# VITA-Group/SinNeRF

Hardware: AMD Instinct MI355X
Metric: rendered rays/sec (64+64 samples), lego 400x400 (higher is better)
Workload: dtype f32; 1 GPU; nerf_synthetic/lego-shaped 400x400 frame (160000 rays/GPU), N_samples=64, N_importance=64, eval render (perturb=0, noise_std=0, white_back), random-init teacher weights; points_per_ray=192, parallelism=rays sharded x1, no collective

## Files before the change

sinnerf_amd/csrc/sn_launch.h:

```cpp
#pragma once
#include <hip/hip_runtime.h>
#include <cstdlib>
#include "../../include/sinnerf_hip.h"
#include "sn_device.h"

namespace snh {

constexpr int MAX_DEVICES = 64;

inline int current_device() {
  int dev = 0;
  if (hipGetDevice(&dev) != hipSuccess || dev < 0 || dev >= MAX_DEVICES) return -1;
  return dev;
}

inline int cu_count() {
  static int cached[MAX_DEVICES];
  const int dev = current_device();
  if (dev < 0) return 256;
  int v = __atomic_load_n(&cached[dev], __ATOMIC_RELAXED);
  if (v == 0) {
    v = 256;
    (void)hipDeviceGetAttribute(&v, hipDeviceAttributeMultiprocessorCount, dev);
    __atomic_store_n(&cached[dev], v, __ATOMIC_RELAXED);
  }
  return v;
}

inline unsigned persistent_grid(long tiles) {
  const int n_cu = cu_count();
  return (unsigned)(tiles < n_cu ? tiles : n_cu);
}

#ifndef SN_DW_NARROW_ASM
#define SN_DW_NARROW_ASM 1
#endif
inline bool narrow_compiler_scheduled() {
  static const bool v = [] { const char* e = getenv("SINNERF_DW_NARROW_COMPILER"); return e != nullptr && e[0] == '1'; }();
  return v;
}
inline bool emb16_refused(int base_dtype, int emb16) {
  return emb16 && (base_dtype != SN_DTYPE_BF16_STATE || !SN_DW_NARROW_ASM || narrow_compiler_scheduled());
}

}

#define SN_ENSURE_DYN_LDS(KFN_, LDS_)                                                                               \
  do {                                                                                                              \
    static int sn_lds_set_[snh::MAX_DEVICES];                                                                       \
    const int sn_dev_ = snh::current_device();                                                                      \
    if (sn_dev_ < 0 || __atomic_load_n(&sn_lds_set_[sn_dev_], __ATOMIC_RELAXED) < (int)(LDS_)) {                    \
      hipError_t sn_e_ = hipFuncSetAttribute(reinterpret_cast<const void*>(KFN_),                                   \
                                             hipFuncAttributeMaxDynamicSharedMemorySize, (int)(LDS_));              \
      if (sn_e_ != hipSuccess) return (int)sn_e_;                                                                   \
      if (sn_dev_ >= 0) __atomic_store_n(&sn_lds_set_[sn_dev_], (int)(LDS_), __ATOMIC_RELAXED);                     \
    }                                                                                                               \
  } while (0)

namespace snd { struct Plan; }
extern "C" {
#define SN_FWD_PARAMS_                                                                                                              \
  const void* blob, const float* in0, const float* in1, long n_points, int s_or_ld, int sigma_only, int input_mode, float* out,    \
      float* acts, float* emb, long slot_rows
#define SN_CHAIN_PARAMS_                                                                                                            \
  const void* bblob, const float* acts, const float* out_raw, const float* g_raw, long n_points, long slot_rows, float* G, float* g_out
#define SN_RAYS_PARAMS_ const void* blob, const float* rays, const float* z_vals, long n_points, int n_samples, float* out
SN_DECLARE_HEADS(sn_mlp_forward_f32, (SN_FWD_PARAMS_, hipStream_t stream));
SN_DECLARE_HEADS(sn_mlp_forward_f32g, (SN_FWD_PARAMS_, hipStream_t stream));
SN_DECLARE_HEADS(sn_mlp_forward_f32g_store, (SN_FWD_PARAMS_, hipStream_t stream));
SN_DECLARE_HEADS(sn_mlp_forward_bf16x3, (SN_FWD_PARAMS_, hipStream_t stream));
SN_DECLARE_HEADS_F16(sn_mlp_forward_bf16, (SN_FWD_PARAMS_, int state_bf16, hipStream_t stream));
SN_DECLARE_HEADS_F16(sn_mlp_forward_bf16_v3, (SN_RAYS_PARAMS_, hipStream_t stream));
SN_DECLARE_HEADS(sn_mlp_forward_bf16_t, (SN_RAYS_PARAMS_, float* acts, float* emb, long slot_rows, int emb16, hipStream_t stream));
SN_DECLARE_HEADS(sn_mlp_forward_bf16x3_t, (SN_RAYS_PARAMS_, float* acts, float* emb, long slot_rows, hipStream_t stream));
SN_DECLARE_HEADS(sn_mlp_backward_chain_f32, (SN_CHAIN_PARAMS_, hipStream_t stream));
SN_DECLARE_HEADS(sn_mlp_backward_chain_f32g, (SN_CHAIN_PARAMS_, hipStream_t stream));
SN_DECLARE_HEADS(sn_mlp_backward_chain_bf16, (SN_CHAIN_PARAMS_, int state_bf16, hipStream_t stream));
SN_DECLARE_HEADS(sn_mlp_backward_chain_bf16_t, (SN_CHAIN_PARAMS_, hipStream_t stream));
SN_DECLARE_HEADS(sn_mlp_backward_chain_bf16x3, (SN_CHAIN_PARAMS_, hipStream_t stream));
SN_DECLARE_HEADS(sn_mlp_backward_chain_bf16x3_t, (SN_CHAIN_PARAMS_, hipStream_t stream));
#undef SN_FWD_PARAMS_
#undef SN_CHAIN_PARAMS_
#undef SN_RAYS_PARAMS_
int sn_dw_launch(const void* tasks, int n_tasks, hipStream_t stream);
long sn_weight_grads_workspace_bytes_impl(long slot_rows, int dtype, int emb16);
int sn_weight_grads_plan_impl(long slot_rows, int dtype, int emb16, int* out, int max_probs);
int sn_weight_grads_launch(const void* acts, const float* emb, const void* G, long slot_rows, int dtype, int emb16, void* workspace,
                           float* const* grads, int accumulate, hipStream_t stream);
int sn_dw_f32_asm_launch(const snd::Plan* plan_host, hipStream_t stream);
int sn_dw_bf16_asm_launch(const snd::Plan* plan_host, hipStream_t stream);
int sn_dw_narrow_bf16_asm_launch(const snd::Plan* plan_host, hipStream_t stream);
int sn_sample_coarse_launch(const float* rays, long n_rays, int n_samples, int use_disp, float perturb,
                            const float* perturb_rand, float* z_out, hipStream_t stream);
int sn_composite_forward_launch(const float* raw, int has_rgb, const float* z_vals, const float* rays,
                                const float* noise, float noise_std, long n_rays, int n_samples, int white_back,
                                float* rgb, float* depth, float* weights, hipStream_t stream);
int sn_composite_backward_launch(const float* raw, const float* z_vals, const float* rays, const float* noise,
                                 float noise_std, long n_rays, int n_samples, int white_back, const float* g_rgb,
                                 const float* g_depth, const float* g_w, float* g_raw, hipStream_t stream);
int sn_composite_backward_rays_launch(const float* raw, const float* z_vals, const float* rays, const float* noise,
                                      float noise_std, long n_rays, int n_samples, int white_back, const float* g_rgb,
                                      const float* g_depth, const float* g_w, float* g_raw, float* g_rays, hipStream_t stream);
int sn_sample_pdf_launch(const float* z_vals, const float* weights, const float* u, long n_rays, int n_samples,
                         int n_importance, float* z_fine, float* z_merged, hipStream_t stream);
int sn_sample_pdf_bins_launch(const float* bins, const float* weights, const float* u, long n_rays, int n_bins,
                              int n_importance, float eps, float* samples, hipStream_t stream);
int sn_generate_rays_launch(const float* c2w, int H, int W, float focal, float near, float far, int x0, int y0, int sx,
                            int sy, int pw, int ph, float* rays, hipStream_t stream);
long sn_generate_rays_backward_workspace_bytes_impl();
int sn_generate_rays_backward_launch(const float* g_rays, int H, int W, float focal, int x0, int y0, int sx, int sy, int pw,
                                     int ph, void* workspace, float* g_c2w, hipStream_t stream);
int sn_generate_rays_cam_launch(const float* c2w, float fx, float fy, float cx, float cy, int convention, int ndc, float ax, float ay,
                                float ndc_near, float near, float far, int x0, int y0, int sx, int sy, int pw, int ph, float* rays,
                                hipStream_t stream);
int sn_generate_rays_cam_backward_launch(const float* g_rays, const float* c2w, float fx, float fy, float cx, float cy, int convention,
                                         int ndc, float ax, float ay, float ndc_near, int x0, int y0, int sx, int sy, int pw, int ph,
                                         void* workspace, float* g_c2w, hipStream_t stream);
int sn_ndc_rays_launch(const float* rays_in, long n_rays, float ax, float ay, float ndc_near, float* rays_out, hipStream_t stream);
int sn_ndc_rays_backward_launch(const float* rays_in, const float* g_rays_out, long n_rays, float ax, float ay, float ndc_near,
                                float* g_rays_in, hipStream_t stream);
int sn_adam_step_launch(float* p, const float* g, float* m, float* v, long n, float lr, float b1, float b2, float eps,
                        float wd, int step, hipStream_t stream);
long sn_render_loss_workspace_bytes_impl();
int sn_render_loss_launch(const float* rgb_c, const float* rgb_f, const float* depth_c, const float* depth_f,
                          const float* rgb_gt, const float* depth_gt, const unsigned char* mask, int mask_mode, long n,
                          float w_rgb, float w_depth, float* g_rgb_c, float* g_rgb_f, float* g_depth_c, float* g_depth_f,
                          void* workspace, float* out, hipStream_t stream);
long sn_ray_grads_workspace_bytes_impl(long n_rays, int n_samples);
int sn_ray_grads_launch(const float* w1, const float* w5, const float* wdir, int layout, const void* g_acts, long slot_rows,
                        const float* rays, const float* z_vals, long n_rays, int n_samples, void* workspace, float* g_rays,
                        hipStream_t stream);
long sn_patch_loss_blocks_impl(int B, int H, int W, int C, int use_ssim);
long sn_patch_loss_workspace_bytes_impl(int B, int H, int W, int C, int use_ssim);
int sn_patch_loss_launch(const float* coarse, const float* fine, const float* target, int B, int H, int W, int C, int use_ssim, int window,
                         float w_mse, float w_ssim, float* g_coarse, float* g_fine, void* workspace, float* out, hipStream_t stream);
long sn_depth_smoothness_workspace_bytes_impl();
int sn_depth_smoothness_launch(const float* idepth, const float* image, int B, int H, int W, int C, float* g_idepth, float* g_image,
                               void* workspace, float* out, hipStream_t stream);
}
```

sinnerf_amd/csrc/sn_mlp_common.h:

```cpp
#pragma once
#include "sn_device.h"
#include "sn_layout.h"
#include "sn_launch.h"

namespace snk {

typedef __attribute__((address_space(3))) void lds_void;
typedef __attribute__((address_space(1))) const void gbl_cvoid;

__device__ __forceinline__ int slab_k_rt(int s) {
  return s < 8 ? snl::K_L0 : s < 32 ? snl::K_HID : s < 40 ? snl::K_SKIP : s < 72 ? snl::K_HID : snl::K_DIR;
}

SN_DEV f32x16 load_bias(const float* lds_bias, int s, int h) {
  const f32x4* p = reinterpret_cast<const f32x4*>(lds_bias + s * 32 + h * 16);
  f32x16 acc;
#pragma unroll
  for (int q = 0; q < 4; ++q) {
    const f32x4 v = p[q];
    acc[4 * q + 0] = v[0]; acc[4 * q + 1] = v[1]; acc[4 * q + 2] = v[2]; acc[4 * q + 3] = v[3];
  }
  return acc;
}

SN_DEV void embed_xyz(float x, float y, float z, int h, float* xe) {
  const Rev2 px = to_revolutions(x), py = to_revolutions(y), pz = to_revolutions(z);
  const float hs = h ? 32.0f : 1.0f;
#pragma unroll
  for (int p = 0; p < 15; ++p) {
    const Rev2 pc = (p % 3 == 0) ? px : (p % 3 == 1) ? py : pz;
    const float scale = hs * (float)(1 << (p / 3));
    sincos_rev(pc, scale, xe[2 * p], xe[2 * p + 1]);
  }
  xe[30] = h ? z : x;
  xe[31] = h ? 0.0f : y;
}
SN_DEV void embed_dir(float x, float y, float z, int h, float* de) {
  const Rev2 px = to_revolutions(x), py = to_revolutions(y), pz = to_revolutions(z);
  const float hs = h ? 4.0f : 1.0f;
#pragma unroll
  for (int p = 0; p < 6; ++p) {
    const Rev2 pc = (p % 3 == 0) ? px : (p % 3 == 1) ? py : pz;
    const float scale = hs * (float)(1 << (p / 3));
    sincos_rev(pc, scale, de[2 * p], de[2 * p + 1]);
  }
  de[12] = h ? z : x;
  de[13] = h ? 0.0f : y;
  de[14] = 0.0f;
  de[15] = 0.0f;
}


constexpr int xyz_col_slot(int k) { return 2 * (3 * (k / 6) + k % 3) + (k % 6) / 3; }
SN_DEV void store_emb_xyz(float* er, const float* f, int h) {
  float* base = er + 3 + 30 * h;
#pragma unroll
  for (int q = 0; q < 7; ++q) {
    f32x4 v;
#pragma unroll
    for (int i = 0; i < 4; ++i) v[i] = f[xyz_col_slot(4 * q + i)];
    __builtin_memcpy(base + 4 * q, &v, 16);
  }
  base[28] = f[xyz_col_slot(28)];
  base[29] = f[xyz_col_slot(29)];
  er[h ? 2 : 0] = f[30];
  if (!h) er[1] = f[31];
}
constexpr int dir_col_slot(int k) { return 2 * (3 * (k / 6) + k % 3) + (k % 6) / 3; }
SN_DEV void store_emb_dir(float* er64, const float* f, int h) {
  float* base = er64 + 3 + 12 * h;
#pragma unroll
  for (int q = 0; q < 3; ++q) {
    f32x4 v;
#pragma unroll
    for (int i = 0; i < 4; ++i) v[i] = f[dir_col_slot(4 * q + i)];
    __builtin_memcpy(base + 4 * q, &v, 16);
  }
  er64[h ? 2 : 0] = f[12];
  if (!h) er64[1] = f[13];
}

SN_DEV void sincos_double(float s, float c, float& s2, float& c2) {
  const float ts = s + s;
  s2 = ts * c;
  c2 = __builtin_fmaf(-ts, s, 1.0f);
}
SN_DEV void embed_xyz_dbl(float x, float y, float z, int h, float* xe) {
  const Rev2 px = to_revolutions(x), py = to_revolutions(y), pz = to_revolutions(z);
  const float hs = h ? 32.0f : 1.0f;
  sincos_rev(px, hs, xe[0], xe[1]);
  sincos_rev(py, hs, xe[2], xe[3]);
  sincos_rev(pz, hs, xe[4], xe[5]);
#pragma unroll
  for (int p = 3; p < 15; ++p) sincos_double(xe[2 * (p - 3)], xe[2 * (p - 3) + 1], xe[2 * p], xe[2 * p + 1]);
  xe[30] = h ? z : x;
  xe[31] = h ? 0.0f : y;
}
SN_DEV void embed_dir_dbl(float x, float y, float z, int h, float* de) {
  const Rev2 px = to_revolutions(x), py = to_revolutions(y), pz = to_revolutions(z);
  const float hs = h ? 4.0f : 1.0f;
  sincos_rev(px, hs, de[0], de[1]);
  sincos_rev(py, hs, de[2], de[3]);
  sincos_rev(pz, hs, de[4], de[5]);
#pragma unroll
  for (int p = 3; p < 6; ++p) sincos_double(de[2 * (p - 3)], de[2 * (p - 3) + 1], de[2 * p], de[2 * p + 1]);
  de[12] = h ? z : x;
  de[13] = h ? 0.0f : y;
  de[14] = 0.0f;
  de[15] = 0.0f;
}
#ifndef SN_EMBED_DBL
#define SN_EMBED_DBL 1
#endif
SN_DEV void embed_xyz_bf16(float x, float y, float z, int h, float* xe) {
  if (SN_EMBED_DBL) embed_xyz_dbl(x, y, z, h, xe); else embed_xyz(x, y, z, h, xe);
}
SN_DEV void embed_dir_bf16(float x, float y, float z, int h, float* de) {
  if (SN_EMBED_DBL) embed_dir_dbl(x, y, z, h, de); else embed_dir(x, y, z, h, de);
}

}
```

sinnerf_amd/csrc/sn_mlp_f32g.h:

```cpp
#pragma once
#include "sn_mlp_pipe.h"
#include <type_traits>

namespace snk {

#ifndef SN_F32G_FD
#define SN_F32G_FD 8
#endif
constexpr int FD_INFER = SN_F32G_FD;
#ifndef SN_F32G_FD_STORE
#define SN_F32G_FD_STORE 16
#endif
constexpr int FD_STORE = SN_F32G_FD_STORE;
constexpr int EPI_STEPS = 24, EPI_STEPS_STORE = 30;
#ifndef SN_F32G_WAIT_G
#define SN_F32G_WAIT_G 6
#endif
constexpr int F32G_LDS_BYTES = TAIL_LDS_BYTES + EPI_LDS_BYTES;
constexpr int F32G_LDS_BYTES_STORE = TAIL_LDS_BYTES + XPOSE_LDS_BYTES;

typedef __amdgpu_buffer_rsrc_t rsrc_t;

SN_DEV f32x4 load_frag(rsrc_t rs, unsigned voff, unsigned soff) {
  typedef unsigned u32x4 __attribute__((ext_vector_type(4)));
  const u32x4 v = __builtin_amdgcn_raw_buffer_load_b128(rs, voff, soff, 0);
  return __builtin_bit_cast(f32x4, v);
}

template <int NG0, int NG1, int SET0, int SET1, int G0, int TOT, int NSTEPS, int FD, class Pending>
SN_DEV void slab_f32g(f32x16& acc, f32x16& accn, f32x4 (&fr)[FD], rsrc_t rs, unsigned voff,
                      const float* bv, const float* lds_bias, int s_next, int h, Pending&& pending) {
  constexpr int NG = NG0 + NG1;
  static_assert(NG % 4 == 0 && TOT % FD == 0 && NG >= 8, "ring index = stream index mod FD");
#pragma unroll
  for (int g = 0; g < NG; ++g) {
    if (g == 0 || g == 12) asm volatile("s_waitcnt lgkmcnt(0)" ::: "memory");
    if (g == 6) accn = load_bias(lds_bias, s_next, h);
    __builtin_amdgcn_sched_barrier(0);
    const f32x4 a_cur = fr[(G0 + g) % FD];
    auto mma = [&](int kk) __attribute__((always_inline)) {
      if (g == 0 && kk == 0) {
        if (SET0 < 0) mma32_v<true>(acc, a_cur[0], bv[0]); else mma32_a<true>(acc, a_cur[0], SET0 * 128);
      } else if (g < NG0) {
        if (SET0 < 0) mma32_v<false>(acc, a_cur[kk], bv[4 * g + kk]); else mma32_a<false>(acc, a_cur[kk], SET0 * 128 + 4 * g + kk);
      } else {
        if (SET1 < 0) mma32_v<false>(acc, a_cur[kk], bv[4 * (g - NG0) + kk]);
        else mma32_a<false>(acc, a_cur[kk], SET1 * 128 + 4 * (g - NG0) + kk);
      }
    };
    auto step = [&](int kk) __attribute__((always_inline)) {
      const int st = 4 * g + kk - 2;
      if (st >= 0 && st < NSTEPS) pending(st);
    };
    mma(0);
    __builtin_amdgcn_sched_barrier(0);
    step(0);
    __builtin_amdgcn_sched_barrier(0);
    mma(1);
    __builtin_amdgcn_sched_barrier(0);
    fr[(G0 + g - 1 + FD) % FD] = load_frag(rs, voff, (unsigned)((G0 + g - 1 + FD) % TOT) * 1024u);
    step(1);
    __builtin_amdgcn_sched_barrier(0);
    mma(2);
    __builtin_amdgcn_sched_barrier(0);
    step(2);
    __builtin_amdgcn_sched_barrier(0);
    mma(3);
    __builtin_amdgcn_sched_barrier(0);
    step(3);
  }
}


}
```

sinnerf_amd/csrc/sn_mlp_fwd_f32g.hip:

```cpp
#include "sn_mlp_f32g.h"

namespace snk {

constexpr unsigned slab_byte_offset(int s) { return (unsigned)(snl::slab_elem_offset(s) * 4); }

template <bool SIGMA_ONLY, int INPUT_MODE, bool STORE>
__global__ void __launch_bounds__(256)
mlp_fwd_f32g_kernel(const char* __restrict__ blob, const float* __restrict__ in0, const float* __restrict__ in1, long P, int S,
                    float* __restrict__ out, float* __restrict__ acts, float* __restrict__ emb, long slot_rows) {
  constexpr int FD = STORE ? FD_STORE : FD_INFER;
  constexpr int NSTEPS = STORE ? EPI_STEPS_STORE : EPI_STEPS;
  extern __shared__ __attribute__((aligned(16))) char smem[];
  float* lds_bias = reinterpret_cast<float*>(smem);
  const float* lds_aux = lds_bias + snl::BIAS_FLOATS;

  const int tid = threadIdx.x;
  const int lane = tid & 63;
  const int wave = tid >> 6;
  const int j = lane & 31;
  const int h = lane >> 5;
  const long n_tiles = (P + 127) / 128;
  constexpr int N_USED = SIGMA_ONLY ? snl::SLAB_FIN : snl::N_SLABS;

  {
    const float4* gb = reinterpret_cast<const float4*>(blob + snl::bias_byte_offset(snl::DT_F32));
    float4* lb = reinterpret_cast<float4*>(lds_bias);
    for (int i = tid; i < snl::TAIL_FLOATS / 4; i += 256) lb[i] = gb[i];
  }
  __syncthreads();

  asm volatile("" ::: "a0", "a255");
  const rsrc_t rs = __builtin_amdgcn_make_buffer_rsrc(const_cast<char*>(blob), 0, (int)snl::blob_bytes(snl::DT_F32), 0x00020000);
  unsigned voff = lane * 16;
  asm volatile("" : "+v"(voff));
  f32x4 fr[FD];
#pragma unroll
  for (int g = 0; g < FD - 1; ++g) fr[g] = load_frag(rs, voff, g * 1024);
  f32x16 acc0 = load_bias(lds_bias, 0, h), acc1;
  char* const xp = smem + TAIL_LDS_BYTES + wave * XPOSE_WAVE_BYTES;
  const unsigned xp_w = (unsigned)(j * XPOSE_PITCH + 4 * h) * 4u;
  const unsigned xp_r = (unsigned)((lane >> 3) * XPOSE_PITCH + 4 * (lane & 7)) * 4u;
  unsigned g_off = (unsigned)((lane >> 3) * 256 + 4 * (lane & 7)) * 4u;
  constexpr int EQ = STORE ? 32 : 1024;
  unsigned epi_a = STORE ? (unsigned)(size_t)xp + xp_w : (unsigned)(size_t)(smem + TAIL_LDS_BYTES + wave * EPI_WAVE_BYTES) + lane * 16;
  asm volatile("" : "+v"(g_off));
  f32x4 rowbuf[2];
  unsigned vzero;
  asm volatile("v_mov_b32 %0, 0" : "=v"(vzero));
  asm volatile("" : "+v"(epi_a));

  for (long tile = blockIdx.x; tile < n_tiles; tile += gridDim.x) {
  const long p_wave = (tile * 4 + __builtin_amdgcn_readfirstlane(wave)) * 32;
  const long p_raw = p_wave + j;
  const bool valid = p_raw < P;
  const long p = valid ? p_raw : P - 1;

  float xe[32];
  if (INPUT_MODE == 0) {
#ifdef SN_F32G_NO_RAY_LOADS
    const float ox = 0.1f, oy = 0.2f, oz = 0.3f, dx = 0.5f, dy = 0.4f, dz = -0.7f, zz = 2.0f + 1e-6f * (float)p;
#else
    const long ray = p / S;
    const float* rp = in0 + ray * 8;
    const float ox = rp[0], oy = rp[1], oz = rp[2], dx = rp[3], dy = rp[4], dz = rp[5];
    const float zz = in1[p];
#endif
    const float x = __fadd_rn(ox, __fmul_rn(dx, zz));
    const float y = __fadd_rn(oy, __fmul_rn(dy, zz));
    const float z = __fadd_rn(oz, __fmul_rn(dz, zz));
#ifdef SN_F32G_NO_VALU_BLOCKS
#pragma unroll
    for (int e = 0; e < 32; ++e) xe[e] = x + (float)e;
#else
    embed_xyz(x, y, z, h, xe);
#endif
  } else {
    const float* row = in0 + p * (long)S;
    int hh = h;
    asm volatile("" : "+v"(hh));
#pragma unroll
    for (int e = 0; e < 32; ++e) {
      const int c0 = snl::xyz_slot_col(0, e), c1 = snl::xyz_slot_col(1, e);
      const int c = hh ? c1 : c0;
      xe[e] = (c >= 0) ? row[c < 0 ? 0 : c] : 0.0f;
    }
  }

  if (STORE && INPUT_MODE == 0) {
    int hh = h;
    asm volatile("" : "+v"(hh));
    store_emb_xyz(emb + p_raw * 128, xe, hh);
  }

  float sg = 0.0f;
  float sv[16];

  auto quad = [](const f32x16& r, int q) __attribute__((always_inline)) {
    f32x4 x;
    x[0] = r[4 * q]; x[1] = r[4 * q + 1]; x[2] = r[4 * q + 2]; x[3] = r[4 * q + 3];
    return x;
  };
  const long p_wave_c = p_wave;
  auto row_read = [&](int i) __attribute__((always_inline)) {
    return *reinterpret_cast<const f32x4*>(xp + xp_r + 8 * i * XPOSE_PITCH * 4);
  };
  auto row_store = [&](int slot, int t, int i, const f32x4& o) __attribute__((always_inline)) {
    const char* base = reinterpret_cast<const char*>(acts) + (((long)slot * slot_rows + p_wave_c + 8 * i) * 256 + 32 * t) * 4;
#ifdef SN_F32G_NO_ROW_STORES
    asm volatile("" :: "v"(o), "s"(base), "v"(g_off));
#else
    __builtin_nontemporal_store(o, reinterpret_cast<f32x4*>(const_cast<char*>(base) + g_off));
#endif
  };
  auto row_step = [&](int slot, int t, int k) __attribute__((always_inline)) {
    if (!STORE) return;
    if (k == 0) rowbuf[0] = row_read(0);
    else if (k == 1) rowbuf[1] = row_read(1);
    else if (k == 2) { row_store(slot, t, 0, rowbuf[0]); rowbuf[0] = row_read(2); }
    else if (k == 3) { row_store(slot, t, 1, rowbuf[1]); rowbuf[1] = row_read(3); }
    else if (k == 4) row_store(slot, t, 2, rowbuf[0]);
    else if (k == 5) row_store(slot, t, 3, rowbuf[1]);
  };
  f32x4 sw[4];
  auto relu_prog = [&](auto wset, auto slot_c, int t, int st, const f32x16& r) __attribute__((always_inline)) {
    constexpr int W = decltype(wset)::value;
    constexpr int slot = decltype(slot_c)::value;
    const int q = st / 6, k = st % 6;
    if (slot == 7) {
      if (st == 0) {
#pragma unroll
        for (int i = 0; i < 4; ++i) sw[i] = *reinterpret_cast<const f32x4*>(lds_aux + snl::AUX_SIGW + h * 128 + 16 * t + 4 * i);
      } else if (st == 3) {
#ifdef SN_F32G_NO_VALU_BLOCKS
#pragma unroll
        for (int i = 0; i < 16; ++i) sv[i] = r[i];
        if (false)
#endif
#pragma unroll
        for (int i = 0; i < 16; ++i) sv[i] = relu1(r[i]);
#pragma unroll
#ifndef SN_F32G_NO_VALU_BLOCKS
        for (int i = 0; i < 16; ++i) sg = __builtin_fmaf(sw[i / 4][i % 4], sv[i], sg);
#else
        for (int i = 0; i < 1; ++i) sg += sv[0];
#endif
        asm volatile("" : "+v"(sg));
      } else if (st >= 4 && st < 8) {
        f32x4 x;
        x[0] = sv[4 * (st - 4)]; x[1] = sv[4 * (st - 4) + 1]; x[2] = sv[4 * (st - 4) + 2]; x[3] = sv[4 * (st - 4) + 3];
        lds_put_quad(epi_a, EQ * (st - 4), x);
      } else if (st >= 8 && st < 12) {
        lds_get_quad_agpr(W * 128 + 16 * t + 4 * (st - 8), epi_a, EQ * (st - 8));
      } else if (st >= 24) {
        row_step(7, t, st - 24);
      }
      return;
    }
    if (st >= 24) { row_step(slot, t, st - 24); return; }
    if (k == 0) lds_put_quad(epi_a, EQ * q, quad(r, q));
#ifndef SN_F32G_NO_ATOMICS
    else if (k < 5) lds_relu_word(epi_a, EQ * q + 4 * (k - 1), vzero);
#endif
    else if (k == 5) lds_get_quad_agpr(W * 128 + 16 * t + 4 * q, epi_a, EQ * q);
  };
  auto copy_prog = [&](auto wset, auto, int t, int st, const f32x16& r) __attribute__((always_inline)) {
    constexpr int W = decltype(wset)::value;
    const int q = st / 6, k = st % 6;
    if (st >= 24) { row_step(8, t, st - 24); return; }
    if (k == 0) lds_put_quad(epi_a, EQ * q, quad(r, q));
    else if (k == 5) lds_get_quad_agpr(W * 128 + 16 * t + 4 * q, epi_a, EQ * q);
  };
  auto no_prog = [&](auto, auto, int, int, const f32x16&) __attribute__((always_inline)) {};

#define SN_C(V_) std::integral_constant<int, V_>{}
#define SN_SLABG(S_, NG0_, NG1_, S0_, S1_, BV_, PEPI_, PW_, PSLOT_, PT_)                                                  \
  do {                                                                                                                    \
    constexpr int s_nx = ((S_) + 1 == N_USED) ? 0 : (S_) + 1;                                                             \
    constexpr int g0 = (int)(slab_byte_offset(S_) / 1024), tot = (int)(slab_byte_offset(N_USED) / 1024);                  \
    if (((S_) & 1) == 0)                                                                                                  \
      slab_f32g<NG0_, NG1_, S0_, S1_, g0, tot, NSTEPS, FD>(acc0, acc1, fr, rs, voff, BV_,                                             \
          lds_bias, s_nx, h, [&](int st) __attribute__((always_inline)) { PEPI_(SN_C(PW_), SN_C(PSLOT_), PT_, st, acc1); }); \
    else                                                                                                                  \
      slab_f32g<NG0_, NG1_, S0_, S1_, g0, tot, NSTEPS, FD>(acc1, acc0, fr, rs, voff, BV_,                                             \
          lds_bias, s_nx, h, [&](int st) __attribute__((always_inline)) { PEPI_(SN_C(PW_), SN_C(PSLOT_), PT_, st, acc0); }); \
  } while (0)
#define SN_LAYERG(L_, NG0_, NG1_, S0_, S1_, EPI_, W_, PEPI_, PW_, PSLOT_)                 \
  do {                                                                                    \
    SN_SLABG(8 * (L_) + 0, NG0_, NG1_, S0_, S1_, xe, PEPI_, PW_, PSLOT_, 7);              \
    SN_SLABG(8 * (L_) + 1, NG0_, NG1_, S0_, S1_, xe, EPI_, W_, L_, 0);                    \
    SN_SLABG(8 * (L_) + 2, NG0_, NG1_, S0_, S1_, xe, EPI_, W_, L_, 1);                    \
    SN_SLABG(8 * (L_) + 3, NG0_, NG1_, S0_, S1_, xe, EPI_, W_, L_, 2);                    \
    SN_SLABG(8 * (L_) + 4, NG0_, NG1_, S0_, S1_, xe, EPI_, W_, L_, 3);                    \
    SN_SLABG(8 * (L_) + 5, NG0_, NG1_, S0_, S1_, xe, EPI_, W_, L_, 4);                    \
    SN_SLABG(8 * (L_) + 6, NG0_, NG1_, S0_, S1_, xe, EPI_, W_, L_, 5);                    \
    SN_SLABG(8 * (L_) + 7, NG0_, NG1_, S0_, S1_, xe, EPI_, W_, L_, 6);                    \
  } while (0)

  SN_LAYERG(0, 8, 0, -1, -1, relu_prog, 0, no_prog, 0, 0);
  SN_LAYERG(1, 32, 0, 0, 0, relu_prog, 1, relu_prog, 0, 0);
  SN_LAYERG(2, 32, 0, 1, 1, relu_prog, 0, relu_prog, 1, 1);
  SN_LAYERG(3, 32, 0, 0, 0, relu_prog, 1, relu_prog, 0, 2);
  SN_LAYERG(4, 8, 32, -1, 1, relu_prog, 0, relu_prog, 1, 3);
  SN_LAYERG(5, 32, 0, 0, 0, relu_prog, 1, relu_prog, 0, 4);
  SN_LAYERG(6, 32, 0, 1, 1, relu_prog, 0, relu_prog, 1, 5);
  SN_LAYERG(7, 32, 0, 0, 0, relu_prog, 1, relu_prog, 0, 6);

  if (SIGMA_ONLY) {
    mfma32_result_fence(acc1);
#pragma unroll
    for (int st = 0; st < EPI_STEPS; ++st) relu_prog(SN_C(1), SN_C(7), 7, st, acc1);
    const float sigma = sg + __shfl_xor(sg, 32, 64) + lds_aux[snl::AUX_HEADB];
    if (valid && h == 0) out[p_raw] = sigma;
    continue;
  }

  SN_LAYERG(8, 32, 0, 1, 1, copy_prog, 0, relu_prog, 1, 7);
  const float sigma = sg + __shfl_xor(sg, 32, 64) + lds_aux[snl::AUX_HEADB];

  float de[16];
  if (INPUT_MODE == 0) {
    const float* rp = in0 + (p / S) * 8;
#ifdef SN_F32G_NO_VALU_BLOCKS
#pragma unroll
    for (int e = 0; e < 16; ++e) de[e] = rp[3] + (float)e;
#else
    embed_dir(rp[3], rp[4], rp[5], h, de);
#endif
  } else {
    const float* row = in0 + p * (long)S;
    int hh = h;
    asm volatile("" : "+v"(hh));
#pragma unroll
    for (int e = 0; e < 16; ++e) {
      const int c0 = snl::dir_slot_col(0, e), c1 = snl::dir_slot_col(1, e);
      const int c = hh ? c1 : c0;
      de[e] = (c >= 0) ? row[63 + (c < 0 ? 0 : c)] : 0.0f;
    }
  }
  if (STORE && INPUT_MODE == 0) {
    int hh = h;
    asm volatile("" : "+v"(hh));
    store_emb_dir(emb + p_raw * 128 + 64, de, hh);
  }
  float c3[3] = {0.0f, 0.0f, 0.0f};
  auto ssp_slice = [&](auto, auto, int t, int st, const f32x16& r) __attribute__((always_inline)) {
    if (st >= 24) { row_step(9, t, st - 24); return; }
    if (st % 6 != 0) return;
    const int q = st / 6;
    float v[4];
#pragma unroll
#ifdef SN_F32G_NO_VALU_BLOCKS
    for (int i = 0; i < 4; ++i) v[i] = r[4 * q + i];
#else
    for (int i = 0; i < 4; ++i) v[i] = SN_NEWACT ? shifted_softplus_fast(r[4 * q + i]) : relu1(r[4 * q + i]);
#endif
#pragma unroll
#ifdef SN_F32G_NO_VALU_BLOCKS
    for (int c = 0; c < 1; ++c) c3[0] += v[0];
    if (false)
#endif
    for (int c = 0; c < 3; ++c) {
      const f32x4 w = *reinterpret_cast<const f32x4*>(lds_aux + snl::AUX_RGBW + c * 128 + h * 64 + 16 * t + 4 * q);
      c3[c] = __builtin_fmaf(w[0], v[0], c3[c]);
      c3[c] = __builtin_fmaf(w[1], v[1], c3[c]);
      c3[c] = __builtin_fmaf(w[2], v[2], c3[c]);
      c3[c] = __builtin_fmaf(w[3], v[3], c3[c]);
    }
    asm volatile("" : "+v"(c3[0]), "+v"(c3[1]), "+v"(c3[2]));
    if (STORE) {
      f32x4 o;
      o[0] = v[0]; o[1] = v[1]; o[2] = v[2]; o[3] = v[3];
      *reinterpret_cast<f32x4*>(xp + xp_w + 32 * q) = o;
    }
  };
  SN_SLABG(72, 32, 4, 0, -1, de, copy_prog, 0, 8, 7);
  SN_SLABG(73, 32, 4, 0, -1, de, ssp_slice, 0, 9, 0);
  SN_SLABG(74, 32, 4, 0, -1, de, ssp_slice, 0, 9, 1);
  SN_SLABG(75, 32, 4, 0, -1, de, ssp_slice, 0, 9, 2);
  mfma32_result_fence(acc1);
#pragma unroll
  for (int q = 0; q < 4; ++q) ssp_slice(SN_C(0), SN_C(9), 3, 6 * q, acc1);
  if (STORE) {
#pragma unroll
    for (int i = 0; i < 4; ++i) row_store(9, 3, i, row_read(i));
  }

  {
    float o3[3];
#pragma unroll
    for (int c = 0; c < 3; ++c) o3[c] = c3[c] + __shfl_xor(c3[c], 32, 64) + lds_aux[snl::AUX_HEADB + 1 + c];
    if (valid && h == 0) {
      float4 o;
      o.x = rgb_activation(o3[0]);
      o.y = rgb_activation(o3[1]);
      o.z = rgb_activation(o3[2]);
      o.w = sigma;
      reinterpret_cast<float4*>(out)[p_raw] = o;
    }
  }
  }
#undef SN_C
#undef SN_SLABG
#undef SN_LAYERG
}

}

#ifdef SN_F32G_TU_STORE
#define SN_F32G_ENTRY sn_mlp_forward_f32g_store
#else
#define SN_F32G_ENTRY sn_mlp_forward_f32g
#endif
#define SN_F32G_LAUNCH_NAME(base) SN_LAUNCH_NAME(base)
extern "C" int SN_F32G_LAUNCH_NAME(SN_F32G_ENTRY)(const void* blob, const float* in0, const float* in1, long n_points, int s_or_ld,
                                             int sigma_only, int input_mode, float* out, float* acts, float* emb, long slot_rows,
                                             hipStream_t stream) {
  using namespace snk;
  if (n_points <= 0) return 0;
  const long tiles = (n_points + 127) / 128;
  const bool store = acts != nullptr;
  if (store && (sigma_only || emb == nullptr || slot_rows < tiles * 128)) return SN_E_BADARG;
  dim3 grid(snh::persistent_grid(tiles)), block(256);
  const size_t lds = store ? F32G_LDS_BYTES_STORE : F32G_LDS_BYTES;
  const char* b = reinterpret_cast<const char*>(blob);
#define SN_LAUNCH(SO, IM, ST)                                                                                       \
  do {                                                                                                              \
    auto kfn = mlp_fwd_f32g_kernel<SO, IM, ST>;                                                                     \
    SN_ENSURE_DYN_LDS(kfn, lds);                                                                                    \
    hipLaunchKernelGGL(kfn, grid, block, lds, stream, b, in0, in1, n_points, s_or_ld, out, acts, emb, slot_rows);   \
  } while (0)
#if defined(SN_F32G_AB)
#ifdef SN_F32G_AB_STORE
  if (!store || input_mode != 0) return SN_E_UNSUPPORTED;
  SN_LAUNCH(false, 0, true);
#else
  if (store || sigma_only || input_mode != 0) return SN_E_UNSUPPORTED;
  SN_LAUNCH(false, 0, false);
#endif
#elif defined(SN_F32G_TU_STORE)
  if (!store) return SN_E_UNSUPPORTED;
  if (input_mode == 0) SN_LAUNCH(false, 0, true); else SN_LAUNCH(false, 1, true);
#elif defined(SN_CLASSIC_HEADS)
  if (store || sigma_only) return SN_E_UNSUPPORTED;
  if (input_mode == 0) SN_LAUNCH(false, 0, false); else SN_LAUNCH(false, 1, false);
#else
  if (store) return SN_E_UNSUPPORTED;
  if (input_mode == 0) { if (sigma_only) SN_LAUNCH(true, 0, false); else SN_LAUNCH(false, 0, false); }
  else { if (sigma_only) SN_LAUNCH(true, 1, false); else SN_LAUNCH(false, 1, false); }
#endif
#undef SN_LAUNCH
  return (int)hipGetLastError();
}
```

Before: 660,900 rays/s.

## Switch f32g inference to per-wave dynamic work stealing with cheaper ray indexing

Replaces the static per-block tile loop with per-wave 32-point units handed out through a global atomic ticket counter that is reset per stream before each launch. The goal is to even out load imbalance across CUs at the tail. It also swaps the 64-bit per-lane p/S division for a per-wave magic-multiply division plus a carry. When a wave's 32 points all share one ray, the direction embedding is computed once across lanes and broadcast through LDS. The cost is an extra memset per launch, an atomic per unit, more LDS, a host-side mutex-guarded map lookup per call, and a hard limit on the number of streams.

Result: faster. 668,500 rays/s, median of 6 (+1.2%).

```diff
diff --git a/sinnerf_amd/csrc/sn_launch.h b/sinnerf_amd/csrc/sn_launch.h
--- a/sinnerf_amd/csrc/sn_launch.h
+++ b/sinnerf_amd/csrc/sn_launch.h
@@ -1,6 +1,8 @@
 #pragma once
 #include <hip/hip_runtime.h>
 #include <cstdlib>
+#include <mutex>
+#include <unordered_map>
 #include "../../include/sinnerf_hip.h"
 #include "sn_device.h"
 
@@ -30,6 +32,21 @@
 inline unsigned persistent_grid(long tiles) {
   const int n_cu = cu_count();
   return (unsigned)(tiles < n_cu ? tiles : n_cu);
+}
+
+constexpr int UNIT_WORDS = 1024;
+inline int unit_word(hipStream_t stream) {
+  static std::mutex mu;
+  static std::unordered_map<hipStream_t, int> of[MAX_DEVICES];
+  const int dev = current_device();
+  if (dev < 0) return -1;
+  std::lock_guard<std::mutex> lock(mu);
+  auto it = of[dev].find(stream);
+  if (it != of[dev].end()) return it->second;
+  const int w = (int)of[dev].size();
+  if (w >= UNIT_WORDS) return -1;
+  of[dev].emplace(stream, w);
+  return w;
 }
 
 #ifndef SN_DW_NARROW_ASM
diff --git a/sinnerf_amd/csrc/sn_mlp_common.h b/sinnerf_amd/csrc/sn_mlp_common.h
--- a/sinnerf_amd/csrc/sn_mlp_common.h
+++ b/sinnerf_amd/csrc/sn_mlp_common.h
@@ -48,6 +48,26 @@
   de[13] = h ? 0.0f : y;
   de[14] = 0.0f;
   de[15] = 0.0f;
+}
+constexpr int DIR_LINE_FLOATS = 32;
+SN_DEV void embed_dir_shared(float x, float y, float z, int lane, float* line, float* de) {
+  const int L = lane < 12 ? lane : 0;
+  const int hh = L >= 6 ? 1 : 0, p = L - 6 * hh, c = p >= 3 ? p - 3 : p;
+  const float v = c == 0 ? x : c == 1 ? y : z;
+  const float scale = (hh ? 4.0f : 1.0f) * (p >= 3 ? 2.0f : 1.0f);
+  float2 sc;
+  sincos_rev(to_revolutions(v), scale, sc.x, sc.y);
+  if (lane < 12) *reinterpret_cast<float2*>(line + 16 * hh + 2 * p) = sc;
+  else if (lane == 12) *reinterpret_cast<float4*>(line + 12) = make_float4(x, y, 0.0f, 0.0f);
+  else if (lane == 13) *reinterpret_cast<float4*>(line + 28) = make_float4(z, 0.0f, 0.0f, 0.0f);
+  __builtin_amdgcn_wave_barrier();
+  const float4* src = reinterpret_cast<const float4*>(line + 16 * (lane >> 5));
+#pragma unroll
+  for (int q = 0; q < 4; ++q) {
+    const float4 t = src[q];
+    de[4 * q] = t.x; de[4 * q + 1] = t.y; de[4 * q + 2] = t.z; de[4 * q + 3] = t.w;
+  }
+  __builtin_amdgcn_wave_barrier();
 }
 
 
diff --git a/sinnerf_amd/csrc/sn_mlp_f32g.h b/sinnerf_amd/csrc/sn_mlp_f32g.h
--- a/sinnerf_amd/csrc/sn_mlp_f32g.h
+++ b/sinnerf_amd/csrc/sn_mlp_f32g.h
@@ -16,7 +16,7 @@
 #ifndef SN_F32G_WAIT_G
 #define SN_F32G_WAIT_G 6
 #endif
-constexpr int F32G_LDS_BYTES = TAIL_LDS_BYTES + EPI_LDS_BYTES;
+constexpr int F32G_LDS_BYTES = TAIL_LDS_BYTES + EPI_LDS_BYTES + 4 * DIR_LINE_FLOATS * 4;
 constexpr int F32G_LDS_BYTES_STORE = TAIL_LDS_BYTES + XPOSE_LDS_BYTES;
 
 typedef __amdgpu_buffer_rsrc_t rsrc_t;
diff --git a/sinnerf_amd/csrc/sn_mlp_fwd_f32g.hip b/sinnerf_amd/csrc/sn_mlp_fwd_f32g.hip
--- a/sinnerf_amd/csrc/sn_mlp_fwd_f32g.hip
+++ b/sinnerf_amd/csrc/sn_mlp_fwd_f32g.hip
@@ -1,13 +1,25 @@
 #include "sn_mlp_f32g.h"
+#include "sn_ray_index.h"
+
+#ifdef SN_F32G_STAMP_EXIT
+#define SN_F32G_STAMP_PARAM , unsigned long* __restrict__ stamp
+#define SN_F32G_STAMP_ARG , sn_f32g_stamp_buffer
+#else
+#define SN_F32G_STAMP_PARAM
+#define SN_F32G_STAMP_ARG
+#endif
 
 namespace snk {
+
+__device__ unsigned f32g_unit_words[snh::UNIT_WORDS];
 
 constexpr unsigned slab_byte_offset(int s) { return (unsigned)(snl::slab_elem_offset(s) * 4); }
 
 template <bool SIGMA_ONLY, int INPUT_MODE, bool STORE>
 __global__ void __launch_bounds__(256)
 mlp_fwd_f32g_kernel(const char* __restrict__ blob, const float* __restrict__ in0, const float* __restrict__ in1, long P, int S,
-                    float* __restrict__ out, float* __restrict__ acts, float* __restrict__ emb, long slot_rows) {
+                    float* __restrict__ out, float* __restrict__ acts, float* __restrict__ emb, long slot_rows,
+                    unsigned unit_word, unsigned long ray_m, unsigned ray_sh SN_F32G_STAMP_PARAM) {
   constexpr int FD = STORE ? FD_STORE : FD_INFER;
   constexpr int NSTEPS = STORE ? EPI_STEPS_STORE : EPI_STEPS;
   extern __shared__ __attribute__((aligned(16))) char smem[];
@@ -19,7 +31,12 @@
   const int wave = tid >> 6;
   const int j = lane & 31;
   const int h = lane >> 5;
-  const long n_tiles = (P + 127) / 128;
+#ifdef SN_F32G_STATIC_UNITS
+  constexpr bool DYN = false;
+#else
+  constexpr bool DYN = !STORE;
+#endif
+  const long n_units = STORE ? (P + 127) / 128 * 4 : (P + 31) / 32;
   constexpr int N_USED = SIGMA_ONLY ? snl::SLAB_FIN : snl::N_SLABS;
 
   {
@@ -34,8 +51,6 @@
   unsigned voff = lane * 16;
   asm volatile("" : "+v"(voff));
   f32x4 fr[FD];
-#pragma unroll
-  for (int g = 0; g < FD - 1; ++g) fr[g] = load_frag(rs, voff, g * 1024);
   f32x16 acc0 = load_bias(lds_bias, 0, h), acc1;
   char* const xp = smem + TAIL_LDS_BYTES + wave * XPOSE_WAVE_BYTES;
   const unsigned xp_w = (unsigned)(j * XPOSE_PITCH + 4 * h) * 4u;
@@ -48,22 +63,52 @@
   unsigned vzero;
   asm volatile("v_mov_b32 %0, 0" : "=v"(vzero));
   asm volatile("" : "+v"(epi_a));
-
-  for (long tile = blockIdx.x; tile < n_tiles; tile += gridDim.x) {
-  const long p_wave = (tile * 4 + __builtin_amdgcn_readfirstlane(wave)) * 32;
+  float* const dir_line = reinterpret_cast<float*>(smem + TAIL_LDS_BYTES + EPI_LDS_BYTES) + wave * DIR_LINE_FLOATS;
+
+#ifdef SN_F32G_STAMP_EXIT
+  const unsigned long t_enter = __builtin_amdgcn_s_memrealtime();
+  unsigned long units_done = 0;
+#endif
+  unsigned* const unit_ctr = f32g_unit_words + unit_word;
+  unsigned ticket = 0, vone = 1;
+  auto request_unit = [&]() __attribute__((always_inline)) {
+    if (lane == 0) asm volatile("s_nop 4\n\tglobal_atomic_add %0, %1, %2, %3 sc0" : "+v"(ticket) : "v"(vzero), "v"(vone), "s"(unit_ctr) : "memory");
+  };
+  if (DYN) request_unit();
+#pragma unroll
+  for (int g = 0; g < FD - 1; ++g) fr[g] = load_frag(rs, voff, g * 1024);
+  const unsigned n_units32 = (unsigned)n_units;
+  for (long unit = (long)blockIdx.x * 4 + __builtin_amdgcn_readfirstlane(wave);; unit += (long)gridDim.x * 4) {
+  if (DYN) {
+    asm volatile("s_waitcnt vmcnt(%1)" : "+v"(ticket) : "n"(FD - 1) : "memory");
+    const unsigned u = (unsigned)__builtin_amdgcn_readfirstlane((int)ticket);
+    if (u >= n_units32) break;
+    unit = (long)u;
+    request_unit();
+  } else if (unit >= n_units) break;
+#ifdef SN_F32G_STAMP_EXIT
+  ++units_done;
+#endif
+  const long p_wave = unit * 32;
   const long p_raw = p_wave + j;
-  const bool valid = p_raw < P;
-  const long p = valid ? p_raw : P - 1;
+  const int j_last = (unsigned)unit + 1u == n_units32 ? (int)((P - 1) & 31) : 31;
+  const bool valid = STORE ? p_raw < P : j <= j_last;
+  const int jc = j < j_last ? j : j_last;
+  const long p = STORE ? (valid ? p_raw : P - 1) : p_wave + jc;
+  const unsigned long ray_w = (!STORE && INPUT_MODE == 0) ? snr::wave_ray((unsigned long)p_wave, ray_m, ray_sh) : 0;
+  const unsigned rem_w = snr::wave_rem((unsigned long)p_wave, ray_w, S);
+  const char* const rays_w = reinterpret_cast<const char*>(in0) + ray_w * 32;
+  unsigned ray_off = 0;
+  if (!STORE && INPUT_MODE == 0) ray_off = snr::lane_carry(rem_w + (unsigned)jc, S) * 32u;
 
   float xe[32];
   if (INPUT_MODE == 0) {
 #ifdef SN_F32G_NO_RAY_LOADS
     const float ox = 0.1f, oy = 0.2f, oz = 0.3f, dx = 0.5f, dy = 0.4f, dz = -0.7f, zz = 2.0f + 1e-6f * (float)p;
 #else
-    const long ray = p / S;
-    const float* rp = in0 + ray * 8;
+    const float* rp = STORE ? in0 + (p / S) * 8 : reinterpret_cast<const float*>(rays_w + ray_off);
     const float ox = rp[0], oy = rp[1], oz = rp[2], dx = rp[3], dy = rp[4], dz = rp[5];
-    const float zz = in1[p];
+    const float zz = STORE ? in1[p] : *reinterpret_cast<const float*>(reinterpret_cast<const char*>(in1 + p_wave) + (unsigned)jc * 4u);
 #endif
     const float x = __fadd_rn(ox, __fmul_rn(dx, zz));
     const float y = __fadd_rn(oy, __fmul_rn(dy, zz));
@@ -210,7 +255,7 @@
 #pragma unroll
     for (int st = 0; st < EPI_STEPS; ++st) relu_prog(SN_C(1), SN_C(7), 7, st, acc1);
     const float sigma = sg + __shfl_xor(sg, 32, 64) + lds_aux[snl::AUX_HEADB];
-    if (valid && h == 0) out[p_raw] = sigma;
+    if (valid && h == 0) (out + p_wave)[j] = sigma;
     continue;
   }
 
@@ -219,12 +264,13 @@
 
   float de[16];
   if (INPUT_MODE == 0) {
-    const float* rp = in0 + (p / S) * 8;
+    const float* rp = STORE ? in0 + (p / S) * 8 : reinterpret_cast<const float*>(rays_w + ray_off);
 #ifdef SN_F32G_NO_VALU_BLOCKS
 #pragma unroll
     for (int e = 0; e < 16; ++e) de[e] = rp[3] + (float)e;
 #else
-    embed_dir(rp[3], rp[4], rp[5], h, de);
+    if (!STORE && rem_w + (unsigned)j_last < (unsigned)S) embed_dir_shared(rp[3], rp[4], rp[5], lane, dir_line, de);
+    else embed_dir(rp[3], rp[4], rp[5], h, de);
 #endif
   } else {
     const float* row = in0 + p * (long)S;
@@ -295,10 +341,21 @@
       o.y = rgb_activation(o3[1]);
       o.z = rgb_activation(o3[2]);
       o.w = sigma;
-      reinterpret_cast<float4*>(out)[p_raw] = o;
-    }
-  }
-  }
+      reinterpret_cast<float4*>(out + 4 * p_wave)[j] = o;
+    }
+  }
+  }
+#ifdef SN_F32G_STAMP_EXIT
+  if (lane == 0) {
+    unsigned xcc;
+    asm volatile("s_getreg_b32 %0, hwreg(HW_REG_XCC_ID)" : "=s"(xcc));
+    unsigned long* rec = stamp + ((long)blockIdx.x * 4 + wave) * 4;
+    rec[0] = t_enter;
+    rec[1] = __builtin_amdgcn_s_memrealtime();
+    rec[2] = xcc & 15u;
+    rec[3] = units_done;
+  }
+#endif
 #undef SN_C
 #undef SN_SLABG
 #undef SN_LAYERG
@@ -312,6 +369,26 @@
 #define SN_F32G_ENTRY sn_mlp_forward_f32g
 #endif
 #define SN_F32G_LAUNCH_NAME(base) SN_LAUNCH_NAME(base)
+#ifdef SN_F32G_STAMP_EXIT
+static unsigned long* sn_f32g_stamp_buffer = nullptr;
+extern "C" void sn_f32g_set_stamp_buffer(unsigned long* device_words) { sn_f32g_stamp_buffer = device_words; }
+#endif
+#if !defined(SN_F32G_TU_STORE) && !defined(SN_F32G_AB_STORE) && !defined(SN_F32G_STATIC_UNITS)
+static int f32g_zeroed_unit_word(hipStream_t stream, unsigned* word) {
+  static unsigned* base[snh::MAX_DEVICES];
+  const int dev = snh::current_device(), w = snh::unit_word(stream);
+  if (dev < 0 || w < 0) return SN_E_UNSUPPORTED;
+  unsigned* b = __atomic_load_n(&base[dev], __ATOMIC_RELAXED);
+  if (b == nullptr) {
+    const hipError_t e = hipGetSymbolAddress(reinterpret_cast<void**>(&b), HIP_SYMBOL(snk::f32g_unit_words));
+    if (e != hipSuccess) return (int)e;
+    __atomic_store_n(&base[dev], b, __ATOMIC_RELAXED);
+  }
+  *word = (unsigned)w;
+  return (int)hipMemsetAsync(b + w, 0, sizeof(unsigned), stream);
+}
+#define SN_F32G_DYNAMIC_UNITS 1
+#endif
 extern "C" int SN_F32G_LAUNCH_NAME(SN_F32G_ENTRY)(const void* blob, const float* in0, const float* in1, long n_points, int s_or_ld,
                                              int sigma_only, int input_mode, float* out, float* acts, float* emb, long slot_rows,
                                              hipStream_t stream) {
@@ -323,11 +400,23 @@
   dim3 grid(snh::persistent_grid(tiles)), block(256);
   const size_t lds = store ? F32G_LDS_BYTES_STORE : F32G_LDS_BYTES;
   const char* b = reinterpret_cast<const char*>(blob);
+  unsigned word = 0;
+  snr::RayDiv rd = {0, 0};
+  if (!store) {
+    if (n_points > snr::MAX_POINTS) return SN_E_TOOLARGE;
+    if (input_mode == 0 && s_or_ld < 1) return SN_E_BADARG;
+    if (input_mode == 0) rd = snr::make_ray_div(s_or_ld);
+#ifdef SN_F32G_DYNAMIC_UNITS
+    const int e = f32g_zeroed_unit_word(stream, &word);
+    if (e != 0) return e;
+#endif
+  }
 #define SN_LAUNCH(SO, IM, ST)                                                                                       \
   do {                                                                                                              \
     auto kfn = mlp_fwd_f32g_kernel<SO, IM, ST>;                                                                     \
     SN_ENSURE_DYN_LDS(kfn, lds);                                                                                    \
-    hipLaunchKernelGGL(kfn, grid, block, lds, stream, b, in0, in1, n_points, s_or_ld, out, acts, emb, slot_rows);   \
+    hipLaunchKernelGGL(kfn, grid, block, lds, stream, b, in0, in1, n_points, s_or_ld, out, acts, emb, slot_rows,    \
+                       word, (unsigned long)rd.m, (unsigned)rd.sh SN_F32G_STAMP_ARG);                                 \
   } while (0)
 #if defined(SN_F32G_AB)
 #ifdef SN_F32G_AB_STORE
diff --git a/sinnerf_amd/csrc/sn_ray_index.h b/sinnerf_amd/csrc/sn_ray_index.h
--- /dev/null
+++ b/sinnerf_amd/csrc/sn_ray_index.h
@@ -0,0 +1,38 @@
+#pragma once
+#include <stdint.h>
+
+#if defined(__HIPCC__)
+#define SN_RAY_HD __host__ __device__ inline
+#else
+#define SN_RAY_HD inline
+#endif
+
+namespace snr {
+
+constexpr int DIVIDEND_BITS = 40;
+constexpr long MAX_POINTS = ((1L << 31) - 1) * 32;
+static_assert(MAX_POINTS + 32 < (1L << DIVIDEND_BITS), "every p_wave is a valid dividend");
+
+struct RayDiv {
+  uint64_t m;
+  uint32_t sh;
+};
+
+inline RayDiv make_ray_div(int S) {
+  int l = 0;
+  while ((1L << l) < (long)S) ++l;
+  RayDiv d;
+  d.sh = (uint32_t)(DIVIDEND_BITS + l);
+  d.m = (uint64_t)((((unsigned __int128)1) << d.sh) / (unsigned)S) + 1;
+  return d;
+}
+
+SN_RAY_HD uint64_t wave_ray(uint64_t p_wave, uint64_t m, uint32_t sh) {
+  return (uint64_t)((((unsigned __int128)p_wave) * m) >> sh);
+}
+SN_RAY_HD uint32_t wave_rem(uint64_t p_wave, uint64_t q, int S) { return (uint32_t)p_wave - (uint32_t)q * (uint32_t)S; }
+SN_RAY_HD uint32_t lane_carry(uint32_t r_plus_j, int S) {
+  return S >= 32 ? (r_plus_j >= (uint32_t)S ? 1u : 0u) : r_plus_j / (uint32_t)S;
+}
+
+}
```
